# eladhoffer/convNet.pytorch

Hardware: AMD Instinct MI355X
Metric: images/sec ResNet-50 bf16 3x224x224 b=256/GPU training (fwd+bwd+SGD) (higher is better)
Workload: dtype bf16; 1 GPU; ResNet-50 (depth:50) synthetic 3x224x224 b=256/GPU bf16, SGD+momentum, 1 MI355X; global_batch=256, parallelism=dp1

## Files before the change

### convnet.pytorch_amd/csrc/junction.hip

```cpp
#include "cn_common.h"
#include "cn_api_internal.h"
#include <type_traits>

struct JdParams {
  const char* dy;
  const char* w;
  const char* addend;
  const char* bn_y;
  const unsigned char* bn_mask;
  const float* bn_coef;
  char* g;
  float* partial;
  int M, m_per_split, nsplit;
  int co_total;
  int addend_sub, H, W, add_H, add_W;
  FastDiv div_hw, div_w;
  unsigned int dy_bytes, out_bytes, add_bytes, mask_bytes;
};

template <typename T, int KD, int CO>
__global__ __launch_bounds__(512) void jdgrad_kernel(JdParams p) {
  static_assert(sizeof(T) == 2, "16-bit storage");
  constexpr int NCW = CO / 64;
  static_assert(NCW == 4 || NCW == 8, "256 or 512 output channels");
// ... 123 lines not shown
      if (m < m_end) {
        float fv[8], fa[8], yv[8];
        Chunk<T>::unpack(v0, fv);
        Chunk<T>::unpack(ep.a[k], fa);
        Chunk<T>::unpack(ep.y[k], yv);
#pragma unroll
        for (int e = 0; e < 8; ++e) fv[e] += fa[e];
        const unsigned int bits = ep.bits[k];
#pragma unroll
        for (int e = 0; e < 8; ++e) fv[e] = ((bits >> e) & 1u) ? fv[e] : 0.f;
        const u32x4 v = Chunk<T>::pack(fv);
        Chunk<T>::unpack(v, fv);
#pragma unroll
        for (int e = 0; e < 8; ++e) {
          bs1[e] += fv[e];
          bs2[e] = fmaf(fv[e], yv[e], bs2[e]);
        }
        cn_st16(p.g + ((size_t)m * COT + (size_t)cb) * 2, v);
      }
    }
    cn_wave_sync();
  };

  if (m_begin < m_end) {
    Epi cur, nxt;
    load_dy(m_begin);
    load_epi(m_begin, cur);
    int buf = 0;
    for (int mb = m_begin; mb < m_end; mb += BM) {
      store_dy(buf);
      __syncthreads();
      const bool more = mb + BM < m_end;
      if (more) { load_dy(mb + BM); load_epi(mb + BM, nxt); }
      compute(mb, buf, cur);
      if (more) cur = nxt;
      buf ^= 1;
    }
  }
  float r1[8], r2[8];
#pragma unroll
  for (int e = 0; e < 8; ++e) {
    const float mu = p.bn_coef[cb + e], is = p.bn_coef[COT + cb + e];
    r1[e] = bs1[e];
    r2[e] = is * (bs2[e] - mu * bs1[e]);
  }
#pragma unroll
  for (int e = 0; e < 8; ++e)
#pragma unroll
    for (int msk = 8; msk <= 32; msk <<= 1) {
      r1[e] += cn_shfl_xor(r1[e], msk);
      r2[e] += cn_shfl_xor(r2[e], msk);
    }
  __syncthreads();
  float* red = (float*)lds;
  if (lane < 8) {
#pragma unroll
    for (int e = 0; e < 8; ++e) {
      red[(wave * 64 + lane * 8 + e) * 2] = r1[e];
      red[(wave * 64 + lane * 8 + e) * 2 + 1] = r2[e];
    }
  }
  __syncthreads();
  if (tid < CO) {
    const int c = tid, wcol = c / 64, cc = c % 64;
    float a1 = 0.f, a2 = 0.f;
#pragma unroll
// ... 176 lines not shown
    for (int e = 0; e < 8; ++e) {
      dst[cb + e] = r1[e];
      dst[COT + cb + e] = r2[e];
    }
  }
}

static int jd_splits(long long M, int BM) {
  int ns = cn_get_option("jdgrad_splits", 256);
  if (ns < 1) ns = 1;
  const long long stages = (M + BM - 1) / BM;
  if (ns > stages) ns = (int)stages;
  return ns;
}
static int jd_bm(int C) { return C == 256 ? 64 : 32; }
static int jd_plan(long long M, int BM, long long* mps_out, int slices = 1) {
  int ns0 = jd_splits(M, BM);
  if (slices > 1) { ns0 = (ns0 + slices - 1) / slices; if (ns0 < 1) ns0 = 1; }
  long long mps = (M + ns0 - 1) / ns0;
  mps = (mps + BM - 1) / BM * BM;
  if (mps_out != nullptr) *mps_out = mps;
  return (int)((M + mps - 1) / mps);
}

extern "C" int cn_conv2d_dgrad_junction_ok(int C, int K, int dtype) {
  if (dtype != CN_BF16 && dtype != CN_F16) return 0;
  if ((C == 512 || C == 1024) && K == 256) return 1;
  return ((C == 256 && (K == 64 || K == 128)) || (C == 512 && K == 128)) ? 1 : 0;
}
extern "C" int cn_conv2d_dgrad_junction_rows_k(int N, int H, int W, int C, int K) {
  return jd_plan((long long)N * H * W, jd_bm(C), nullptr, K >= 256 ? C / 256 : 1);
}

extern "C" cn_status cn_conv2d_dgrad_junction(const void* dy, const void* w_crsk, void* g, const void* addend, int addend_sub,
                                              int N, int H, int W, int C, int K, int dtype, const void* bn_y,
                                              const unsigned char* bn_mask, const float* bn_coef, float* partial,
                                              int partial_rows, void* stream) {
  if (!cn_conv2d_dgrad_junction_ok(C, K, dtype)) { cn_set_error("conv2d_dgrad_junction: K=%d -> C=%d dtype %d is not an instantiated shape", K, C, dtype); return CN_ESHAPE; }
  if (dy == nullptr || w_crsk == nullptr || g == nullptr || addend == nullptr || bn_y == nullptr || bn_mask == nullptr ||
      bn_coef == nullptr || partial == nullptr) { cn_set_error("conv2d_dgrad_junction: null operand"); return CN_EINVAL; }
  if (addend_sub != 1 && addend_sub != 2) { cn_set_error("conv2d_dgrad_junction: addend subsampling %d (1 or 2)", addend_sub); return CN_EINVAL; }
  const long long M = (long long)N * H * W;
  if (M <= 0) { cn_set_error("conv2d_dgrad_junction: empty"); return CN_ESHAPE; }
  const long long ob = M * C * 2, db = M * K * 2;
  const int aH = (H + 1) / 2, aW = (W + 1) / 2;
  const long long ab = addend_sub == 2 ? (long long)N * aH * aW * C * 2 : ob;
  if (ob >= (1ll << 31) || db >= (1ll << 31)) { cn_set_error("conv2d_dgrad_junction: operand exceeds the 2 GiB buffer-descriptor window"); return CN_ESHAPE; }
  const int BM = jd_bm(C);
  const bool w32 = K >= 256;
  long long mps = 0;
  const int nsplit = jd_plan(M, BM, &mps, w32 ? C / 256 : 1);
  if (partial_rows < nsplit) { cn_set_error("conv2d_dgrad_junction: partial buffer of %d rows < %d", partial_rows, nsplit); return CN_EWORKSPACE; }
  JdParams p;
  memset(&p, 0, sizeof(p));
  p.dy = (const char*)dy; p.w = (const char*)w_crsk; p.addend = (const char*)addend; p.bn_y = (const char*)bn_y;
  p.bn_mask = bn_mask; p.bn_coef = bn_coef; p.g = (char*)g; p.partial = partial;
  p.M = (int)M; p.m_per_split = (int)mps; p.nsplit = nsplit;
  p.co_total = C;
  p.addend_sub = addend_sub; p.H = H; p.W = W; p.add_H = aH; p.add_W = aW;
  p.div_hw = cn_make_fastdiv((unsigned)(H * W)); p.div_w = cn_make_fastdiv((unsigned)W);
  p.dy_bytes = (unsigned int)db; p.out_bytes = (unsigned int)ob; p.add_bytes = (unsigned int)ab;
  hipStream_t st = (hipStream_t)stream;
  const char* tn = dtype == CN_F16 ? "f16_t" : "bf16_t";
  if (w32) {
    cn_set_last_kernel("jdgrad_w32_kernel<%s, %d> [%d channels]", tn, K, C);
    dim3 g32((unsigned)nsplit, (unsigned)(C / 256));
    if (dtype == CN_F16) CN_LAUNCH((jdgrad_w32_kernel<f16_t, 256>), g32, dim3(512), st, p);
    else CN_LAUNCH((jdgrad_w32_kernel<bf16_t, 256>), g32, dim3(512), st, p);
    return cn_check_launch("jdgrad_w32");
  }
  cn_set_last_kernel("jdgrad_kernel<%s, %d, %d>", tn, K, C);
  dim3 grid((unsigned)nsplit, (unsigned)(C > 512 ? C / 512 : 1));
#define JD_GO(KD, CO)                                                                           \
  do {                                                                                          \
    if (dtype == CN_F16) CN_LAUNCH((jdgrad_kernel<f16_t, KD, CO>), grid, dim3(512), st, p);      \
    else CN_LAUNCH((jdgrad_kernel<bf16_t, KD, CO>), grid, dim3(512), st, p);                     \
  } while (0)
  if (C == 256 && K == 64) JD_GO(64, 256);
  else if (C == 256 && K == 128) JD_GO(128, 256);
  else JD_GO(128, 512);
#undef JD_GO
  return cn_check_launch("jdgrad");
}

struct JfParams {
  const char* x;
  const char* w;
  char* y;
  float* partial;
  int M, m_per_split, nsplit;
  int co_total;
  unsigned int x_bytes;
  const float* xf;
  char* a_out;
  int relu;
};

template <typename T, int KD, int CO, bool XF = false>
__global__ __launch_bounds__(512) void jfwd_kernel(JfParams p) {
  static_assert(sizeof(T) == 2, "16-bit storage");
  constexpr int NCW = CO / 64;
  static_assert(NCW == 4 || NCW == 8, "256 or 512 output channels");
  constexpr int PH = 8 / NCW;
  constexpr int BM = 32 * PH;
  constexpr int NKK = KD / 16;
  constexpr int NCD = KD / 8;
  constexpr int DYB = BM * KD * 2;
  constexpr int ND = BM * NCD / 512;
  static_assert(ND >= 1 && BM * NCD % 512 == 0, "x tile staging");
  constexpr int PP = 144;
  constexpr int PRIV = 32 * PP;
  __shared__ __attribute__((aligned(16))) char lds[2 * DYB + 8 * PRIV];
  const int tid = threadIdx.x;
  const int lane = tid & 63;
  const int wave = cn_uniform(tid >> 6);
// ... 352 lines not shown
```

### convnet.pytorch_amd/flags.py

```python
import os

INFINITY_CACHE_BYTES = 256 * 2 ** 20
LAZY_MIN_BYTES = 0.6 * INFINITY_CACHE_BYTES

_DEFAULTS = {
    'fuse_bn_stats': 1,
    'fuse_bn_bwd': 1,
    'fuse_stem_pool': 1,
    'stem_xmax': 1,
    'subsampled_shortcut_grad': 1,
    'dual_bn': 1,
    'lazy_dy': 1,
    'lazy_min_mb': LAZY_MIN_BYTES / 2 ** 20,
    'lazy_z': 1,
    'lazy_a': '1',
    'jpair': 1,
    'jpair_recompute': 1,
    'jdgrad': 1,
    'centered_stats': '1',
    'stem_pairs': 1, 'stem_halo': 1, 'conv3x3_halo': 1, 'conv1x1_stream': 1,
    'dwconv': 1,
    'wgrad_stream': 1,
    'side_hold': 1,
    'dgrad_first': 1,
    'marks': 1,
    'main_stream_prio': '-1',
    'graph': 'auto',
    'graph_dp': 0,
    'plan': 1,
    'quant_int8': 0,
    'quant_fuse': 1,
    'quant_qp_from_producer': 1,
    'quant_store8': 1,
    'quant_wgrad_side': 1,
    'quant_junction_add': 1,
}

_ENV = 'CONVNET_AMD_FLAGS'


def _parse():
    vals = dict(_DEFAULTS)
    for item in os.environ.get(_ENV, '').split(','):
        item = item.strip()
        if not item:
            continue
        name, _, v = item.partition('=')
        if name not in vals:
            raise ValueError('%s: unknown flag %r (known: %s)' % (_ENV, name, ', '.join(sorted(vals))))
        vals[name] = v
    return vals
# ... 28 lines not shown
```

### convnet.pytorch_amd/ops.py

```python
import collections
import contextlib
import os
import typing
import weakref

import torch
import torch.distributed as dist
from torch.autograd import Function

from . import _lib, flags
from ._lib import dtype_code, ptr, stream_of

_WS = {}


def workspace(nbytes, device, tag='main'):
    dev = torch.device(device)
    sid = torch.cuda.current_stream(dev).cuda_stream if dev.type == 'cuda' else 0
    key = (str(dev), tag, sid)
    buf = _WS.get(key)
    if buf is None or buf.numel() * 4 < nbytes:
        n = max(int(nbytes + 3) // 4, 1024)
        old = buf
        buf = torch.empty(n, dtype=torch.float32, device=dev)
# ... 180 lines not shown
def conv_out_hw(H, W, R, S, stride, pad):
    return (H + 2 * pad[0] - R) // stride[0] + 1, (W + 2 * pad[1] - S) // stride[1] + 1



FUSE_BN_STATS = flags.on('fuse_bn_stats')
STEM_PAIRS = flags.on('stem_pairs')
STEM_HALO = flags.on('stem_halo')
CONV3X3_HALO = flags.on('conv3x3_halo')
CONV1X1_STREAM = flags.on('conv1x1_stream')
FUSE_STEM_POOL = flags.on('fuse_stem_pool')
FUSE_BN_BWD = flags.on('fuse_bn_bwd')
LAZY_DY = flags.on('lazy_dy')
LAZY_DY_MIN_MB = float(flags.get('lazy_min_mb'))
DUAL_BN = flags.on('dual_bn')
LAZY_Z = flags.on('lazy_z')
LAZY_Z_MIN_MB = float(flags.get('lazy_min_mb'))
LAZY_Z_SCOPE = [0]
JPAIR = flags.on('jpair')
JPAIR_RECOMPUTE = flags.on('jpair_recompute')
_BN_Y_PRODUCER = [None]


@contextlib.contextmanager
def bn_y_is_output_of(w_krsc):
    prev, _BN_Y_PRODUCER[0] = _BN_Y_PRODUCER[0], w_krsc
    try:
        yield
    finally:
        _BN_Y_PRODUCER[0] = prev


JDGRAD = flags.on('jdgrad')
DGRAD_FIRST = flags.on('dgrad_first')


COUNTERS = {'bn_fwd_fused': 0, 'bn_fwd_plain': 0, 'bn_bwd_fused': 0, 'bn_bwd_plain': 0, 'bn_bwd_lazy': 0}


class _PendingStats(object):
    __slots__ = ('partial', 'rows', 'pivot')


def _stats_partial(want, K, device, rows_fn, *dims):
    if not want:
        return None, 0
    rows = rows_fn(*dims)
    return torch.empty((rows, 2 * K), dtype=torch.float32, device=device), rows


def _park_stats(y, partial, rows, pivot=None):
    if partial is None:
        return
    ps = _PendingStats()
    ps.partial, ps.rows = partial, rows
    ps.pivot = pivot.data_ptr() if pivot is not None else None
    y._cn_stats = ps


def take_pending_stats(y):
    ps = getattr(y, '_cn_stats', None)
    if ps is not None:
        del y._cn_stats
    return ps


# ... 180 lines not shown
            and conv.out_channels <= 128 and conv.in_channels <= 512 and conv.training
            and not getattr(conv, 'out_f32', False))


def conv2d_dgrad(dy, w_crsk, x_shape, K, R, S, stride, pad, addend=None, bn=None, addend_sub=1):
    N, H, W, C = x_shape
    dx = torch.empty((N, H, W, C), dtype=dy.dtype, device=dy.device)
    name = _last_kernel()
    detail = _conv_detail('dgrad', C, H, K, R, stride)
    flops = 2.0 * dy.numel() * C * R * S
    nbytes = dy.numel() * _esize(dy) + dx.numel() * _esize(dx) + K * R * S * C * _esize(dy) \
        + (addend.numel() * _esize(addend) if addend is not None else 0)
    if addend is not None and addend_sub == 2:
        assert tuple(addend.shape) == (N, (H + 1) // 2, (W + 1) // 2, C), 'subsampled addend shape'
    if bn is None and addend is None and _halo3x3_ok(dy, K, C, R, S, stride, pad) and tuple(dy.shape[1:3]) == (H, W):
        PROFILER.run(name, 1, flops, nbytes,
                     lambda: _L().cn_conv3x3_c64(ptr(dy), ptr(w_crsk), ptr(dx), N, H, W, dtype_code(dy.dtype), 1, None,
                                                 0, stream_of(dy)),
                     dy.device, detail=detail)
        return dx
    if bn is None:
        PROFILER.run(name, stride[0] * stride[1], flops, nbytes,
                     lambda: _L().cn_conv2d_dgrad_sa(ptr(dy), ptr(w_crsk), ptr(dx), ptr(addend), int(addend_sub), N, H,
                                                     W, C, K, R, S, stride[0], stride[1], pad[0], pad[1],
                                                     dtype_code(dy.dtype), 0, stream_of(dy)),
                     dy.device, detail=detail)
        return dx
    bn_y, bn_mask, bn_stats, bn_relu = BnBwdOperands(*bn)
    L = _L()
    if JDGRAD and (R, S) == (1, 1) and tuple(stride) == (1, 1) and tuple(pad) == (0, 0) and bn_mask is not None \
            and addend is not None and L.cn_conv2d_dgrad_junction_ok(C, K, dtype_code(dy.dtype)):
        rows = L.cn_conv2d_dgrad_junction_rows_k(N, H, W, C, K)
        partial = torch.empty((rows, 2 * C), dtype=torch.float32, device=dy.device)
        PROFILER.run(_last_kernel(), 1, flops, nbytes + dx.numel() * _esize(dx) + partial.numel() * 4,
                     lambda: L.cn_conv2d_dgrad_junction(ptr(dy), ptr(w_crsk), ptr(dx), ptr(addend), int(addend_sub), N,
                                                        H, W, C, K, dtype_code(dy.dtype), ptr(bn_y), ptr(bn_mask),
                                                        ptr(bn_stats), ptr(partial), rows, stream_of(dy)),
                     dy.device, detail=detail)
        COUNTERS['jdgrad'] = COUNTERS.get('jdgrad', 0) + 1
        return dx, partial, rows
    rows = L.cn_conv2d_dgrad_bnbwd_rows(N, H, W, C, stride[0], stride[1])
    partial = torch.empty((rows, 2 * C), dtype=torch.float32, device=dy.device)
    PROFILER.run(name, stride[0] * stride[1], flops, nbytes + dx.numel() * _esize(dx) + partial.numel() * 4,
                 lambda: L.cn_conv2d_dgrad_bnbwd_sa(ptr(dy), ptr(w_crsk), ptr(dx), ptr(addend), int(addend_sub), N, H,
                                                    W, C, K, R, S, stride[0], stride[1], pad[0], pad[1],
                                                    dtype_code(dy.dtype), ptr(bn_y), ptr(bn_mask), ptr(bn_stats),
                                                    int(bn_relu), ptr(partial), rows, stream_of(dy)),
                 dy.device, detail=detail)
    return dx, partial, rows


def _wgrad_two_phase(call, device, flops, bytes_partial, bytes_reduce, detail, suffix=''):
    if not (PROFILER.enabled and device.type == 'cuda'):
        return call()
    L = _L()
    L.cn_set_option(b'wgrad_phase', 1)
    try:
        PROFILER.run(_last_kernel(suffix), 1, flops, bytes_partial, call, device, detail=detail)
        L.cn_set_option(b'wgrad_phase', 2)
        PROFILER.run('wgrad_reduce_kernel', 1, 0.0, bytes_reduce, call, device, detail=detail + ' [reduce]')
    finally:
        L.cn_set_option(b'wgrad_phase', 0)


def conv2d_wgrad(x, dy, dw_krsc, c_real, K, R, S, stride, pad, beta=1.0, scale=1.0, tag='main'):
    N, H, W, C = x.shape
    code = dtype_code(x.dtype)
    L = _L()
    need = L.cn_conv2d_wgrad_workspace(N, H, W, C, K, R, S, stride[0], stride[1], pad[0], pad[1], code)
    ws = workspace(need, x.device, tag)

# ... 325 lines not shown
    _L().cn_cast_from_f32(ptr(x), ptr(y), x.numel(), dtype_code(dtype), stream_of(x))
    return y


def fill_f32_(x, v=0.0):
    _L().cn_fill_f32(ptr(x), x.numel(), float(v), stream_of(x))
    return x



def _input_bn_state(conv_mod, x):
    bn_mod = getattr(conv_mod, 'input_bn', None)
    if bn_mod is None:
        return None
    ref = getattr(bn_mod, '_fwd_ctx', None)
    bctx = ref() if ref is not None else None
    if bctx is None or getattr(bctx, 'out_ptr', None) != x.data_ptr():
        return None
    try:
        saved = bctx.saved_tensors
    except RuntimeError:
        return None
    y, stats = saved[0], saved[1]
    mask = saved[2] if len(saved) > 2 else None
    if tuple(y.shape) != tuple(x.shape) or y.dtype != x.dtype:
        return None
    if bctx.has_res and bctx.relu and mask is None:
        return None
    if y.shape[-1] % _lib.chunk_elems(y.dtype) != 0:
        return None
    return bn_mod, BnBwdOperands(y, mask, stats, bctx.relu)


_ZEROS = {}


def _zero_like_placeholder(x):
    key = (x.device, x.dtype)
    z = _ZEROS.get(key)
    if z is None:
        z = _ZEROS[key] = torch.zeros(1, dtype=x.dtype, device=x.device)
    return z.expand(x.shape)


def _is_zero_placeholder(t):
    z = _ZEROS.get((t.device, t.dtype))
    return z is not None and t.data_ptr() == z.data_ptr() and t.dim() > 0 and all(st == 0 for st in t.stride())


def _submit_wgrad(mod, run, held, dy):
    x = held[0]
    if SIDE.active(x):
        SIDE.submit(x.device, lambda: held + (run('side') or ()), mod._notify_grad_ready, dy)
    else:
        run('main')
        mod._notify_grad_ready()


class Conv2dFunction(Function):
    @staticmethod
    def forward(ctx, x, weight, bias, mod):
        mod.ensure_prepared()
        lz, la = _take(mod, '_lazy_z', x), _take(mod, '_lazy_a', x)
        if bias is not None and (lz is not None or la is not None):
            raise _lib.ConvNetHipError(_MISMATCH['_lazy_z' if lz is not None else '_lazy_a'])
        if lz is not None:
            y = conv2d_fwd_lazyz(lz, mod.w_krsc, mod.out_channels, bn_stats=_wants_stats(mod), pivot=stats_pivot(mod))
            COUNTERS['lazy_z'] = COUNTERS.get('lazy_z', 0) + 1
        elif la is not None:
            y = conv2d_fwd_lazya(la, mod.w_krsc, mod.out_channels, bn_stats=_wants_stats(mod), kernel=mod.kernel_size)
            COUNTERS['lazy_a'] = COUNTERS.get('lazy_a', 0) + 1
        else:
            y = conv2d_fwd(x, mod.w_krsc, bias, mod.out_channels, mod.kernel_size[0], mod.kernel_size[1],
                           mod.stride, mod.padding, out_f32=mod.out_f32, bn_stats=_wants_stats(mod),
                           pivot=stats_pivot(mod))
        ctx.mod = mod
        ctx.has_bias = bias is not None
        ctx.save_for_backward(x)
        ctx.out_key = _owner_key(y)
        _take(mod, '_lazy_dy')
        return y

    @staticmethod
    def backward(ctx, dy):
        (x,) = ctx.saved_tensors
        mod = ctx.mod
        lazy = _take(mod, '_lazy_dy', ctx.out_key)
        holder = getattr(mod, '_res_holder', None)
        R, S = mod.kernel_size
        if lazy is None and _is_zero_placeholder(dy):
            raise _lib.ConvNetHipError('lazy dy: the gradient placeholder reached a convolution with an empty mailbox '
                                       '(the BatchNorm that parked the gradient is not this convolution\'s consumer)')
        if lazy is not None:
            g, bn_y, coef = lazy
            if tuple(g.shape) != tuple(dy.shape):
                raise _lib.ConvNetHipError(_MISMATCH['_lazy_dy'])
            if JPAIR and (R, S) == (1, 1) and mod.stride == (1, 1) and mod.padding == (0, 0) and ctx.needs_input_grad[0] \
                    and mod.in_channels == x.shape[-1] \
                    and _L().cn_conv2d_bwd1x1_lazy_ok(x.shape[-1], mod.out_channels, dtype_code(x.dtype)):
                if holder is not None and holder.dres is not None:
                    raise _lib.ConvNetHipError('lazy dy met a fused-addend dgrad: the junction layout changed')
                own = JPAIR_RECOMPUTE and not ctx.has_bias and _owner_key(bn_y) == ctx.out_key
                with bn_y_is_output_of(mod.w_krsc if own else None):
                    dx = conv2d_bwd1x1_lazy(x, g, bn_y, coef, mod.w_crsk, mod.grad_view('weight'), mod.out_channels)
                mod._notify_grad_ready()
                COUNTERS['jpair'] = COUNTERS.get('jpair', 0) + 1
                if holder is not None:
                    holder.park(dx)
                return dx, None, None, None
            _submit_wgrad(mod, lambda tag: conv2d_wgrad_lazy(x, g, bn_y, coef, mod.grad_view('weight'), mod.in_channels,
                                                             mod.out_channels, R, S, mod.stride, mod.padding, tag=tag),
                          (x, g, bn_y, coef), coef)
            if not ctx.needs_input_grad[0]:
# ... 12 lines not shown
                holder.park(dx)
            return dx, None, None, None
        dy = dy.contiguous()
        if dy.dtype != x.dtype:
            dy = cast_from_f32(dy, x.dtype)
        if ctx.has_bias:
            colsum(dy.view(-1, mod.out_channels), mod.grad_view('bias'))

        def submit_wgrad():
            _submit_wgrad(mod, lambda tag: conv2d_wgrad(x, dy, mod.grad_view('weight'), mod.in_channels, mod.out_channels,
                                                        R, S, mod.stride, mod.padding, tag=tag), (x, dy), dy)

        def dgrad_part():
            dx = None
            if ctx.needs_input_grad[0]:
                addend, addend_sub = None, 1
                if holder is not None and holder.dres is not None and holder.dres.dtype == dy.dtype \
                        and (holder.dres.shape == x.shape if holder.sub == 1 else
                             tuple(holder.dres.shape) == (x.shape[0], (x.shape[1] + 1) // 2, (x.shape[2] + 1) // 2, x.shape[3])):
                    addend, addend_sub = holder.claim()
                elif holder is not None and holder.dres is None and SUBSAMPLED_SHORTCUT_GRAD \
                        and (R, S) == (1, 1) and mod.stride == (2, 2) and mod.padding == (0, 0):
                    N_, H_, W_, C_ = x.shape
                    compact = conv2d_dgrad(dy, mod.w_crsk, (N_, (H_ + 1) // 2, (W_ + 1) // 2, C_), mod.out_channels, 1, 1,
                                           (1, 1), (0, 0))
                    holder.park(compact, 2)
                    return _zero_like_placeholder(x), None, None, None
                final = holder is None or addend is not None
                bn_args = _input_bn_state(mod, x) if (final and FUSE_BN_BWD) else None
                if bn_args is not None and holder is None:
                    bn_args = None
                if bn_args is not None:
                    bn_mod, bn = bn_args
                    dx, partial, rows = conv2d_dgrad(dy, mod.w_crsk, x.shape, mod.out_channels, R, S, mod.stride,
                                                     mod.padding, addend=addend, bn=bn, addend_sub=addend_sub)
                    _park(bn_mod, '_bwd_partials', dx, BwdPartials(partial, rows))
                else:
                    dx = conv2d_dgrad(dy, mod.w_crsk, x.shape, mod.out_channels, R, S, mod.stride, mod.padding,
                                      addend=addend, addend_sub=addend_sub)
                if holder is not None and addend is None:
                    holder.park(dx)
            return dx, None, None, None

        if not DGRAD_FIRST:
            submit_wgrad()
        out = dgrad_part()
        if DGRAD_FIRST:
            submit_wgrad()
        return out


class GroupedConv2dFunction(Function):
    @staticmethod
    def forward(ctx, x, weight, mod):
        mod.ensure_prepared()
        _refuse_parked(mod, 'grouped convolution')
        y = gconv2d_fwd(x, mod.w_krsc, mod.out_channels, mod.groups, mod.stride[0])
        ctx.mod = mod
        ctx.save_for_backward(x)
        COUNTERS['gconv'] = COUNTERS.get('gconv', 0) + 1
        return y

    @staticmethod
    def backward(ctx, dy):
        (x,) = ctx.saved_tensors
        mod = ctx.mod
        _refuse_parked(mod, 'grouped convolution')
        if _is_zero_placeholder(dy):
# ... 845 lines not shown
```

### include/convnet_hip.h

```cpp
#ifndef CONVNET_HIP_H
#define CONVNET_HIP_H
#include <stddef.h>
#ifdef __cplusplus
extern "C" {
#endif

#define CN_OK 0
#define CN_EINVAL (-1)
#define CN_ESHAPE (-2)
#define CN_EHIP (-3)
#define CN_EWORKSPACE (-4)
#define CN_ERCCL (-5)
#define CN_F32 0
#define CN_BF16 1
#define CN_F16 2
typedef int cn_status;

const char* cn_last_error(void);
const char* cn_build_info(void);
const char* cn_last_kernel_name(void);
const char* cn_kernel_log(int clear);
int cn_is_emulator(void);
int cn_set_option(const char* name, int value);
cn_status cn_stream_fork(void* from_stream, void* to_stream);
// ... 31 lines not shown
cn_status cn_conv3x3_c64_lazya(const void* bn_y, const float* stats, int relu, void* a_out, const void* w, void* y, int N, int H,
                               int W, int dtype, float* partial, int partial_rows, void* stream);
int cn_stem_fwd_ok(int K, int R, int S2, int Jp, int dtype);
int cn_stem_fwd_rows(int N, int P);
cn_status cn_stem_fwd(const void* xp, const void* wp, void* y, int N, int Hp, int Jp, int dtype, float* partial,
                      int partial_rows, void* stream);
int cn_stem_wgrad_ok(int K, int R, int S2, int Jp, int dtype);
size_t cn_stem_wgrad_workspace(int N, int Hp);
cn_status cn_stem_wgrad(const void* xp, const void* dy, float* dwp, int N, int Hp, int Jp, int dtype, float beta, float scale,
                        void* workspace, size_t ws_bytes, void* stream);
cn_status cn_conv2d_fwd_lazyz(const void* bn_y, const void* res, const float* stats, const float* res_stats, int relu, void* z,
                              unsigned char* z_mask, const void* w_krsc, void* y, int N, int H, int W, int C, int K, int dtype,
                              float* partial, int partial_rows, const float* pivot, void* stream);
int cn_conv2d_dgrad_bnbwd_rows(int N, int H, int W, int C, int stride_h, int stride_w);
cn_status cn_conv2d_dgrad_sa(const void* dy, const void* w_crsk, void* dx, const void* addend, int addend_sub, int N, int H,
                             int W, int C, int K, int R, int S, int stride_h, int stride_w, int pad_h, int pad_w, int dtype,
                             int out_f32, void* stream);
cn_status cn_conv2d_dgrad_bnbwd_sa(const void* dy, const void* w_crsk, void* g, const void* addend, int addend_sub, int N,
                                   int H, int W, int C, int K, int R, int S, int stride_h, int stride_w, int pad_h, int pad_w,
                                   int dtype, const void* bn_y, const unsigned char* bn_mask, const float* bn_coef,
                                   int bn_relu, float* partial, int partial_rows, void* stream);
int cn_conv1x1_stream_fwd_ok(int C, int K, int dtype);
int cn_conv1x1_stream_fwd_rows(int N, int H, int W, int K);
cn_status cn_conv1x1_stream_fwd(const void* x, const void* w_krsc, void* y, int N, int H, int W, int C, int K, int dtype,
                                float* partial, int partial_rows, void* stream);
cn_status cn_conv1x1_stream_fwd_lazya(const void* bn_y, const float* stats, int relu, void* a_out, const void* w_krsc, void* y,
                                      int N, int H, int W, int C, int K, int dtype, float* partial, int partial_rows,
                                      void* stream);
int cn_conv2d_dgrad_junction_ok(int C, int K, int dtype);
int cn_conv2d_dgrad_junction_rows_k(int N, int H, int W, int C, int K);
cn_status cn_conv2d_dgrad_junction(const void* dy, const void* w_crsk, void* g, const void* addend, int addend_sub, int N, int H,
                                   int W, int C, int K, int dtype, const void* bn_y, const unsigned char* bn_mask,
                                   const float* bn_coef, float* partial, int partial_rows, void* stream);
int cn_gconv2d_ok(int C, int K, int groups, int R, int S, int stride_h, int stride_w, int pad_h, int pad_w, int dtype);
cn_status cn_gconv2d_fwd(const void* x, const void* w, void* y, int N, int H, int W, int C, int K, int groups, int stride,
                         int dtype, void* stream);
cn_status cn_gconv2d_dgrad(const void* dy, const void* w, void* dx, int N, int H, int W, int C, int K, int groups, int stride,
                           int dtype, void* stream);
size_t cn_gconv2d_wgrad_workspace(int N, int H, int W, int C, int K, int groups, int stride, int dtype);
cn_status cn_gconv2d_wgrad(const void* x, const void* dy, float* dw, int N, int H, int W, int C, int K, int groups, int stride,
                           int dtype, float beta, float scale, void* workspace, size_t ws_bytes, void* stream);
int cn_dwconv3x3_ok(int C, int R, int S, int stride_h, int stride_w, int pad_h, int pad_w, int dtype);
cn_status cn_dwconv3x3_fwd(const void* x, const void* w_rsc, const float* bias, void* y, int N, int H, int W, int C, int stride,
                           int dtype, void* stream);
cn_status cn_dwconv3x3_dgrad(const void* dy, const void* w_rsc, void* dx, int N, int H, int W, int C, int stride, int dtype,
                             void* stream);
size_t cn_dwconv3x3_wgrad_workspace(int N, int H, int W, int C, int stride, int dtype);
cn_status cn_dwconv3x3_wgrad(const void* x, const void* dy, float* dw, float* dbias, int N, int H, int W, int C, int stride,
                             int dtype, float beta, float scale, void* workspace, size_t ws_bytes, void* stream);
size_t cn_conv2d_wgrad_workspace(int N, int H, int W, int C, int K, int R, int S, int stride_h, int stride_w,
                                 int pad_h, int pad_w, int dtype);
cn_status cn_conv2d_wgrad(const void* x, const void* dy, float* dw_krsc, int C_real, int N, int H, int W, int C,
                          int K, int R, int S, int stride_h, int stride_w, int pad_h, int pad_w, int dtype,
                          float beta, float scale, void* workspace, size_t ws_bytes, void* stream);
cn_status cn_conv2d_dgrad_lazy(const void* g, const void* bn_y, const float* coef, const void* w_crsk, void* dx, int N, int H,
                               int W, int C, int K, int R, int S, int stride_h, int stride_w, int pad_h, int pad_w, int dtype,
                               void* stream);
cn_status cn_conv2d_wgrad_lazy(const void* x, const void* g, const void* bn_y, const float* coef, float* dw_krsc, int C_real,
                               int N, int H, int W, int C, int K, int R, int S, int stride_h, int stride_w, int pad_h,
                               int pad_w, int dtype, float beta, float scale, void* workspace, size_t ws_bytes, void* stream);
int cn_conv2d_dgrad_lazy_stream_ok(int C, int K, int dtype);
cn_status cn_conv2d_dgrad_lazy_stream(const void* g, const void* bn_y, const float* coef, const void* w_crsk, void* dx, int N,
                                      int H, int W, int C, int K, int dtype, void* stream);
int cn_conv2d_bwd1x1_lazy_ok(int C, int K, int dtype);
size_t cn_conv2d_bwd1x1_lazy_workspace(int N, int H, int W, int C, int K);
cn_status cn_conv2d_bwd1x1_lazy(const void* x, const void* g, const void* bn_y, const float* coef, const void* w_crsk, void* dx,
// ... 244 lines not shown
```

Baseline: 15080 images/sec.

## Recompute BN input from 1x1 producer conv inside junction dgrad kernel

Adds a jdgrad_kernel_ry variant that recomputes the BatchNorm input y on the fly as a 1x1 convolution of the saved 64-channel producer input, instead of reading the stored 256-channel bn_y tensor. The Python side detects when the BN's producer is a bias-free 1x1 conv with 64 input channels and routes through the new path by default. This trades extra MFMA work and LDS staging of the producer weights for reading a narrower tensor from HBM. It also lets bn_y avoid being materialized or read in the backward pass for those layers.

```diff
diff --git a/convnet.pytorch_amd/csrc/junction.hip b/convnet.pytorch_amd/csrc/junction.hip
--- a/convnet.pytorch_amd/csrc/junction.hip
+++ b/convnet.pytorch_amd/csrc/junction.hip
@@ -179,6 +179,287 @@
       __syncthreads();
       const bool more = mb + BM < m_end;
       if (more) { load_dy(mb + BM); load_epi(mb + BM, nxt); }
+      compute(mb, buf, cur);
+      if (more) cur = nxt;
+      buf ^= 1;
+    }
+  }
+  float r1[8], r2[8];
+#pragma unroll
+  for (int e = 0; e < 8; ++e) {
+    const float mu = p.bn_coef[cb + e], is = p.bn_coef[COT + cb + e];
+    r1[e] = bs1[e];
+    r2[e] = is * (bs2[e] - mu * bs1[e]);
+  }
+#pragma unroll
+  for (int e = 0; e < 8; ++e)
+#pragma unroll
+    for (int msk = 8; msk <= 32; msk <<= 1) {
+      r1[e] += cn_shfl_xor(r1[e], msk);
+      r2[e] += cn_shfl_xor(r2[e], msk);
+    }
+  __syncthreads();
+  float* red = (float*)lds;
+  if (lane < 8) {
+#pragma unroll
+    for (int e = 0; e < 8; ++e) {
+      red[(wave * 64 + lane * 8 + e) * 2] = r1[e];
+      red[(wave * 64 + lane * 8 + e) * 2 + 1] = r2[e];
+    }
+  }
+  __syncthreads();
+  if (tid < CO) {
+    const int c = tid, wcol = c / 64, cc = c % 64;
+    float a1 = 0.f, a2 = 0.f;
+#pragma unroll
+    for (int g2 = 0; g2 < PH; ++g2) {
+      a1 += red[((g2 * NCW + wcol) * 64 + cc) * 2];
+      a2 += red[((g2 * NCW + wcol) * 64 + cc) * 2 + 1];
+    }
+    float* dst = p.partial + (size_t)split * 2 * COT;
+    dst[co0 + c] = a1;
+    dst[COT + co0 + c] = a2;
+  }
+}
+
+struct JdRyParams {
+  JdParams j;
+  const char* px;
+  const char* pw;
+  unsigned int px_bytes;
+};
+
+template <typename T, int KD, int CO, int KX>
+__global__ __launch_bounds__(512) void jdgrad_kernel_ry(JdRyParams q) {
+  static_assert(sizeof(T) == 2, "16-bit storage");
+  const JdParams& p = q.j;
+  constexpr int NCW = CO / 64;
+  static_assert(NCW == 4 || NCW == 8, "256 or 512 output channels");
+  constexpr int PH = 8 / NCW;
+  constexpr int BM = 32 * PH;
+  constexpr int NKK = KD / 16;
+  constexpr int NCD = KD / 8;
+  constexpr int DYB = BM * KD * 2;
+  constexpr int ND = BM * NCD / 512;
+  static_assert(ND >= 1 && BM * NCD % 512 == 0, "dy tile staging");
+  constexpr int NKX = KX / 16;
+  constexpr int NCX = KX / 8;
+  constexpr int XB = BM * KX * 2;
+  constexpr int NX = BM * NCX / 512;
+  static_assert(NX >= 1 && BM * NCX % 512 == 0 && NCX >= 8, "px tile staging");
+  constexpr int PP = 144;
+  constexpr int PRIV = 32 * PP;
+  constexpr bool WL = KD > 64;
+  constexpr int WLB = WL ? CO * KX * 2 : 0;
+  __shared__ __attribute__((aligned(16))) char lds[2 * DYB + 2 * XB + 8 * PRIV + WLB];
+  const int tid = threadIdx.x;
+  const int lane = tid & 63;
+  const int wave = cn_uniform(tid >> 6);
+  const int cw = wave % NCW, ph = wave / NCW;
+  const int h = lane >> 5;
+  char* xt = lds + 2 * DYB;
+  char* priv = lds + 2 * DYB + 2 * XB + wave * PRIV;
+  char* wl = lds + 2 * DYB + 2 * XB + 8 * PRIV;
+
+  const int split = blockIdx.x;
+  const int co0 = blockIdx.y * CO, COT = p.co_total;
+  const int m_begin = split * p.m_per_split;
+  int m_end = m_begin + p.m_per_split;
+  if (m_end > p.M) m_end = p.M;
+
+  s16x8 wf[2][NKK], wy[2][WL ? 1 : NKX];
+#pragma unroll
+  for (int t = 0; t < 2; ++t) {
+    const int c = co0 + cw * 64 + t * 32 + (lane & 31);
+#pragma unroll
+    for (int kk = 0; kk < NKK; ++kk)
+      wf[t][kk] = __builtin_bit_cast(s16x8, cn_ld16(p.w + ((size_t)c * KD + 16 * kk + 8 * h) * 2));
+    if constexpr (!WL) {
+#pragma unroll
+      for (int kk = 0; kk < NKX; ++kk)
+        wy[t][kk] = __builtin_bit_cast(s16x8, cn_ld16(q.pw + ((size_t)c * KX + 16 * kk + 8 * h) * 2));
+    }
+  }
+  if constexpr (WL) {
+    for (int id = tid; id < CO * NCX; id += 512) {
+      const int row = id / NCX, c = id - row * NCX;
+      const int cs = NCX == 8 ? (c ^ ((row >> 1) & 7)) : (c ^ (row & (NCX - 1)));
+      cn_st16(wl + row * (KX * 2) + (cs << 4), cn_ld16(q.pw + ((size_t)(co0 + row) * KX + (size_t)c * 8) * 2));
+    }
+  }
+
+  const cn_buf_t dybuf = cn_make_buf(p.dy, p.dy_bytes);
+  const cn_buf_t abuf = cn_make_buf(p.addend, p.add_bytes);
+  const cn_buf_t xbuf = cn_make_buf(q.px, q.px_bytes);
+  const int ech = lane & 7, erow = lane >> 3;
+  const int cb = co0 + cw * 64 + ech * 8;
+  const int HW = p.H * p.W;
+
+  struct Epi {
+    u32x4 a[4];
+    unsigned int bits[4];
+  };
+  u32x4 dreg[ND], xreg[NX];
+  auto load_tiles = [&](int mb) {
+#pragma unroll
+    for (int i = 0; i < ND; ++i) {
+      const int id = tid + 512 * i;
+      const int row = id / NCD, c = id - row * NCD;
+      const int m = mb + row;
+      dreg[i] = cn_buf_ld16(dybuf, m < m_end ? ((unsigned int)m * (unsigned int)KD + (unsigned int)c * 8u) * 2u : CN_OOB);
+    }
+#pragma unroll
+    for (int i = 0; i < NX; ++i) {
+      const int id = tid + 512 * i;
+      const int row = id / NCX, c = id - row * NCX;
+      const int m = mb + row;
+      xreg[i] = cn_buf_ld16(xbuf, m < m_end ? ((unsigned int)m * (unsigned int)KX + (unsigned int)c * 8u) * 2u : CN_OOB);
+    }
+  };
+  auto load_epi = [&](int mb, Epi& e) {
+#pragma unroll
+    for (int k = 0; k < 4; ++k) {
+      const int m = mb + ph * 32 + k * 8 + erow;
+      const bool ok = m < m_end;
+      unsigned int oa = ok ? ((unsigned int)m * (unsigned int)COT + (unsigned int)cb) * 2u : CN_OOB;
+      if (p.addend_sub == 2) {
+        const int mm = ok ? m : 0;
+        const int n = (int)cn_fastdiv((unsigned)mm, p.div_hw);
+        const int rem = mm - n * HW;
+        const int ho = (int)cn_fastdiv((unsigned)rem, p.div_w);
+        const int wo = rem - ho * p.W;
+        const bool even = ((ho | wo) & 1) == 0;
+        const int apx = (n * p.add_H + (ho >> 1)) * p.add_W + (wo >> 1);
+        oa = (ok && even) ? ((unsigned int)apx * (unsigned int)COT + (unsigned int)cb) * 2u : CN_OOB;
+      }
+      e.a[k] = cn_buf_ld16(abuf, oa);
+      e.bits[k] = ok ? (unsigned int)p.bn_mask[(size_t)m * (COT / 8) + (cb >> 3)] : 0u;
+    }
+  };
+  auto store_tiles = [&](int buf) {
+    char* t = lds + buf * DYB;
+#pragma unroll
+    for (int i = 0; i < ND; ++i) {
+      const int id = tid + 512 * i;
+      const int row = id / NCD, c = id - row * NCD;
+      const int cs = NCD == 8 ? (c ^ ((row >> 1) & 7)) : (c ^ (row & (NCD - 1)));
+      cn_st16(t + row * (KD * 2) + (cs << 4), dreg[i]);
+    }
+    char* u = xt + buf * XB;
+#pragma unroll
+    for (int i = 0; i < NX; ++i) {
+      const int id = tid + 512 * i;
+      const int row = id / NCX, c = id - row * NCX;
+      const int cs = NCX == 8 ? (c ^ ((row >> 1) & 7)) : (c ^ (row & (NCX - 1)));
+      cn_st16(u + row * (KX * 2) + (cs << 4), xreg[i]);
+    }
+  };
+
+  float bs1[8], bs2[8];
+#pragma unroll
+  for (int e = 0; e < 8; ++e) { bs1[e] = 0.f; bs2[e] = 0.f; }
+
+  auto compute = [&](int mb, int buf, const Epi& ep) {
+    const int prow = ph * 32 + (lane & 31);
+    f32x16 acc[2];
+#pragma unroll
+    for (int x = 0; x < 2; ++x)
+#pragma unroll
+      for (int r = 0; r < 16; ++r) acc[x][r] = 0.f;
+    {
+      const char* rowp = lds + buf * DYB + prow * (KD * 2);
+      const int sw = NCD == 8 ? ((prow >> 1) & 7) : (prow & (NCD - 1));
+#pragma unroll
+      for (int kk = 0; kk < NKK; ++kk) {
+        const s16x8 b = __builtin_bit_cast(s16x8, cn_ld16(rowp + (((2 * kk + h) ^ sw) << 4)));
+#pragma unroll
+        for (int x = 0; x < 2; ++x) {
+          if constexpr (std::is_same<T, f16_t>::value) acc[x] = cn_mfma_32x32x16_f16(wf[x][kk], b, acc[x]);
+          else acc[x] = cn_mfma_32x32x16_bf16(wf[x][kk], b, acc[x]);
+        }
+      }
+    }
+    auto to_patch = [&]() {
+#pragma unroll
+      for (int x = 0; x < 2; ++x)
+#pragma unroll
+        for (int q4 = 0; q4 < 4; ++q4) {
+          u32x2 pk;
+          pk[0] = cn_pack2<T>(acc[x][q4 * 4], acc[x][q4 * 4 + 1]);
+          pk[1] = cn_pack2<T>(acc[x][q4 * 4 + 2], acc[x][q4 * 4 + 3]);
+          *(u32x2*)(priv + (lane & 31) * PP + (x * 32 + 8 * q4 + 4 * h) * 2) = pk;
+        }
+    };
+    to_patch();
+    cn_wave_sync();
+    u32x4 v0[4];
+#pragma unroll
+    for (int k = 0; k < 4; ++k) v0[k] = cn_ld16(priv + (k * 8 + erow) * PP + ech * 16);
+    cn_wave_sync();
+#pragma unroll
+    for (int x = 0; x < 2; ++x)
+#pragma unroll
+      for (int r = 0; r < 16; ++r) acc[x][r] = 0.f;
+    {
+      const char* rowp = xt + buf * XB + prow * (KX * 2);
+      const int sw = NCX == 8 ? ((prow >> 1) & 7) : (prow & (NCX - 1));
+#pragma unroll
+      for (int kk = 0; kk < NKX; ++kk) {
+        const s16x8 b = __builtin_bit_cast(s16x8, cn_ld16(rowp + (((2 * kk + h) ^ sw) << 4)));
+#pragma unroll
+        for (int x = 0; x < 2; ++x) {
+          s16x8 a;
+          if constexpr (WL) {
+            const int wrow = cw * 64 + x * 32 + (lane & 31);
+            const int ws = NCX == 8 ? ((wrow >> 1) & 7) : (wrow & (NCX - 1));
+            a = __builtin_bit_cast(s16x8, cn_ld16(wl + wrow * (KX * 2) + (((2 * kk + h) ^ ws) << 4)));
+          } else {
+            a = wy[x][kk];
+          }
+          if constexpr (std::is_same<T, f16_t>::value) acc[x] = cn_mfma_32x32x16_f16(a, b, acc[x]);
+          else acc[x] = cn_mfma_32x32x16_bf16(a, b, acc[x]);
+        }
+      }
+    }
+    to_patch();
+    cn_wave_sync();
+#pragma unroll
+    for (int k = 0; k < 4; ++k) {
+      const int m = mb + ph * 32 + k * 8 + erow;
+      const u32x4 y0 = cn_ld16(priv + (k * 8 + erow) * PP + ech * 16);
+      if (m < m_end) {
+        float fv[8], fa[8], yv[8];
+        Chunk<T>::unpack(v0[k], fv);
+        Chunk<T>::unpack(ep.a[k], fa);
+        Chunk<T>::unpack(y0, yv);
+#pragma unroll
+        for (int e = 0; e < 8; ++e) fv[e] += fa[e];
+        const unsigned int bits = ep.bits[k];
+#pragma unroll
+        for (int e = 0; e < 8; ++e) fv[e] = ((bits >> e) & 1u) ? fv[e] : 0.f;
+        const u32x4 v = Chunk<T>::pack(fv);
+        Chunk<T>::unpack(v, fv);
+#pragma unroll
+        for (int e = 0; e < 8; ++e) {
+          bs1[e] += fv[e];
+          bs2[e] = fmaf(fv[e], yv[e], bs2[e]);
+        }
+        cn_st16(p.g + ((size_t)m * COT + (size_t)cb) * 2, v);
+      }
+    }
+    cn_wave_sync();
+  };
+
+  if (m_begin < m_end) {
+    Epi cur, nxt;
+    load_tiles(m_begin);
+    load_epi(m_begin, cur);
+    int buf = 0;
+    for (int mb = m_begin; mb < m_end; mb += BM) {
+      store_tiles(buf);
+      __syncthreads();
+      const bool more = mb + BM < m_end;
+      if (more) { load_tiles(mb + BM); load_epi(mb + BM, nxt); }
       compute(mb, buf, cur);
       if (more) cur = nxt;
       buf ^= 1;
@@ -421,12 +702,12 @@
   return jd_plan((long long)N * H * W, jd_bm(C), nullptr, K >= 256 ? C / 256 : 1);
 }
 
-extern "C" cn_status cn_conv2d_dgrad_junction(const void* dy, const void* w_crsk, void* g, const void* addend, int addend_sub,
-                                              int N, int H, int W, int C, int K, int dtype, const void* bn_y,
-                                              const unsigned char* bn_mask, const float* bn_coef, float* partial,
-                                              int partial_rows, void* stream) {
+static cn_status jd_run(const void* dy, const void* w_crsk, void* g, const void* addend, int addend_sub, int N, int H, int W,
+                        int C, int K, int dtype, const void* bn_y, const void* prod_x, const void* prod_w_krsc, int KX,
+                        const unsigned char* bn_mask, const float* bn_coef, float* partial, int partial_rows, void* stream) {
+  const bool ry = bn_y == nullptr;
   if (!cn_conv2d_dgrad_junction_ok(C, K, dtype)) { cn_set_error("conv2d_dgrad_junction: K=%d -> C=%d dtype %d is not an instantiated shape", K, C, dtype); return CN_ESHAPE; }
-  if (dy == nullptr || w_crsk == nullptr || g == nullptr || addend == nullptr || bn_y == nullptr || bn_mask == nullptr ||
+  if (dy == nullptr || w_crsk == nullptr || g == nullptr || addend == nullptr || (ry && (prod_x == nullptr || prod_w_krsc == nullptr)) || bn_mask == nullptr ||
       bn_coef == nullptr || partial == nullptr) { cn_set_error("conv2d_dgrad_junction: null operand"); return CN_EINVAL; }
   if (addend_sub != 1 && addend_sub != 2) { cn_set_error("conv2d_dgrad_junction: addend subsampling %d (1 or 2)", addend_sub); return CN_EINVAL; }
   const long long M = (long long)N * H * W;
@@ -434,7 +715,7 @@
   const long long ob = M * C * 2, db = M * K * 2;
   const int aH = (H + 1) / 2, aW = (W + 1) / 2;
   const long long ab = addend_sub == 2 ? (long long)N * aH * aW * C * 2 : ob;
-  if (ob >= (1ll << 31) || db >= (1ll << 31)) { cn_set_error("conv2d_dgrad_junction: operand exceeds the 2 GiB buffer-descriptor window"); return CN_ESHAPE; }
+  if (ob >= (1ll << 31) || db >= (1ll << 31) || (ry && M * KX * 2 >= (1ll << 31))) { cn_set_error("conv2d_dgrad_junction: operand exceeds the 2 GiB buffer-descriptor window"); return CN_ESHAPE; }
   const int BM = jd_bm(C);
   const bool w32 = K >= 256;
   long long mps = 0;
@@ -451,6 +732,22 @@
   p.dy_bytes = (unsigned int)db; p.out_bytes = (unsigned int)ob; p.add_bytes = (unsigned int)ab;
   hipStream_t st = (hipStream_t)stream;
   const char* tn = dtype == CN_F16 ? "f16_t" : "bf16_t";
+  if (ry) {
+    JdRyParams q;
+    memset(&q, 0, sizeof(q));
+    q.j = p; q.px = (const char*)prod_x; q.pw = (const char*)prod_w_krsc; q.px_bytes = (unsigned int)(M * KX * 2);
+    cn_set_last_kernel("jdgrad_kernel_ry<%s, %d, %d, %d>", tn, K, C, KX);
+    dim3 grid((unsigned)nsplit);
+#define JD_GO(KD, CO, KXX)                                                                         \
+  do {                                                                                             \
+    if (dtype == CN_F16) CN_LAUNCH((jdgrad_kernel_ry<f16_t, KD, CO, KXX>), grid, dim3(512), st, q); \
+    else CN_LAUNCH((jdgrad_kernel_ry<bf16_t, KD, CO, KXX>), grid, dim3(512), st, q);                \
+  } while (0)
+    if (K == 64) JD_GO(64, 256, 64);
+    else JD_GO(128, 256, 64);
+#undef JD_GO
+    return cn_check_launch("jdgrad_ry");
+  }
   if (w32) {
     cn_set_last_kernel("jdgrad_w32_kernel<%s, %d> [%d channels]", tn, K, C);
     dim3 g32((unsigned)nsplit, (unsigned)(C / 256));
@@ -470,6 +767,27 @@
   else JD_GO(128, 512);
 #undef JD_GO
   return cn_check_launch("jdgrad");
+}
+extern "C" cn_status cn_conv2d_dgrad_junction(const void* dy, const void* w_crsk, void* g, const void* addend, int addend_sub,
+                                              int N, int H, int W, int C, int K, int dtype, const void* bn_y,
+                                              const unsigned char* bn_mask, const float* bn_coef, float* partial,
+                                              int partial_rows, void* stream) {
+  if (bn_y == nullptr) { cn_set_error("conv2d_dgrad_junction: null operand"); return CN_EINVAL; }
+  return jd_run(dy, w_crsk, g, addend, addend_sub, N, H, W, C, K, dtype, bn_y, nullptr, nullptr, 0, bn_mask, bn_coef, partial,
+                partial_rows, stream);
+}
+extern "C" int cn_conv2d_dgrad_junction_ry_ok(int C, int K, int KX, int dtype) {
+  if (dtype != CN_BF16 && dtype != CN_F16) return 0;
+  return (C == 256 && (K == 64 || K == 128) && KX == 64) ? 1 : 0;
+}
+extern "C" cn_status cn_conv2d_dgrad_junction_ry(const void* dy, const void* w_crsk, void* g, const void* addend, int addend_sub,
+                                                 int N, int H, int W, int C, int K, int KX, int dtype, const void* prod_x,
+                                                 const void* prod_w_krsc, const unsigned char* bn_mask, const float* bn_coef,
+                                                 float* partial, int partial_rows, void* stream) {
+  if (!cn_conv2d_dgrad_junction_ry_ok(C, K, KX, dtype)) { cn_set_error("conv2d_dgrad_junction_ry: K=%d -> C=%d from KX=%d dtype %d is not an instantiated shape", K, C, KX, dtype); return CN_ESHAPE; }
+  if (prod_x == nullptr || prod_w_krsc == nullptr) { cn_set_error("conv2d_dgrad_junction_ry: null operand"); return CN_EINVAL; }
+  return jd_run(dy, w_crsk, g, addend, addend_sub, N, H, W, C, K, dtype, nullptr, prod_x, prod_w_krsc, KX, bn_mask, bn_coef,
+                partial, partial_rows, stream);
 }
 
 struct JfParams {
diff --git a/convnet.pytorch_amd/flags.py b/convnet.pytorch_amd/flags.py
--- a/convnet.pytorch_amd/flags.py
+++ b/convnet.pytorch_amd/flags.py
@@ -17,6 +17,7 @@
     'jpair': 1,
     'jpair_recompute': 1,
     'jdgrad': 1,
+    'jdgrad_recompute': 1,
     'centered_stats': '1',
     'stem_pairs': 1, 'stem_halo': 1, 'conv3x3_halo': 1, 'conv1x1_stream': 1,
     'dwconv': 1,
diff --git a/convnet.pytorch_amd/ops.py b/convnet.pytorch_amd/ops.py
--- a/convnet.pytorch_amd/ops.py
+++ b/convnet.pytorch_amd/ops.py
@@ -236,6 +236,19 @@
 
 
 JDGRAD = flags.on('jdgrad')
+JDGRAD_RECOMPUTE = flags.on('jdgrad_recompute')
+_BN_Y_CONV1X1 = [None]
+
+
+@contextlib.contextmanager
+def bn_y_is_conv1x1_of(prod_x, prod_w_krsc):
+    prev, _BN_Y_CONV1X1[0] = _BN_Y_CONV1X1[0], (prod_x, prod_w_krsc) if prod_x is not None else None
+    try:
+        yield
+    finally:
+        _BN_Y_CONV1X1[0] = prev
+
+
 DGRAD_FIRST = flags.on('dgrad_first')
 
 
@@ -482,11 +495,28 @@
             and addend is not None and L.cn_conv2d_dgrad_junction_ok(C, K, dtype_code(dy.dtype)):
         rows = L.cn_conv2d_dgrad_junction_rows_k(N, H, W, C, K)
         partial = torch.empty((rows, 2 * C), dtype=torch.float32, device=dy.device)
-        PROFILER.run(_last_kernel(), 1, flops, nbytes + dx.numel() * _esize(dx) + partial.numel() * 4,
-                     lambda: L.cn_conv2d_dgrad_junction(ptr(dy), ptr(w_crsk), ptr(dx), ptr(addend), int(addend_sub), N,
-                                                        H, W, C, K, dtype_code(dy.dtype), ptr(bn_y), ptr(bn_mask),
-                                                        ptr(bn_stats), ptr(partial), rows, stream_of(dy)),
-                     dy.device, detail=detail)
+        prod = _BN_Y_CONV1X1[0]
+        if prod is not None and L.cn_conv2d_dgrad_junction_ry_ok(C, K, prod[0].shape[-1], dtype_code(dy.dtype)):
+            px, pw = prod
+            KX = px.shape[-1]
+            if px.numel() != N * H * W * KX or pw.numel() != C * KX or px.dtype != dy.dtype or pw.dtype != dy.dtype \
+                    or not px.is_contiguous() or not pw.is_contiguous():
+                raise _lib.ConvNetHipError('conv2d_dgrad: bn_y_is_conv1x1_of operands do not describe a %d -> %d channel '
+                                           '1x1 convolution over this input' % (KX, C))
+            PROFILER.run(_last_kernel(), 1, flops + 2.0 * px.numel() * C,
+                         nbytes + (px.numel() + pw.numel()) * _esize(px) + partial.numel() * 4,
+                         lambda: L.cn_conv2d_dgrad_junction_ry(ptr(dy), ptr(w_crsk), ptr(dx), ptr(addend), int(addend_sub),
+                                                               N, H, W, C, K, KX, dtype_code(dy.dtype), ptr(px), ptr(pw),
+                                                               ptr(bn_mask), ptr(bn_stats), ptr(partial), rows,
+                                                               stream_of(dy)),
+                         dy.device, detail=detail)
+            COUNTERS['jdgrad_ry'] = COUNTERS.get('jdgrad_ry', 0) + 1
+        else:
+            PROFILER.run(_last_kernel(), 1, flops, nbytes + dx.numel() * _esize(dx) + partial.numel() * 4,
+                         lambda: L.cn_conv2d_dgrad_junction(ptr(dy), ptr(w_crsk), ptr(dx), ptr(addend), int(addend_sub), N,
+                                                            H, W, C, K, dtype_code(dy.dtype), ptr(bn_y), ptr(bn_mask),
+                                                            ptr(bn_stats), ptr(partial), rows, stream_of(dy)),
+                         dy.device, detail=detail)
         COUNTERS['jdgrad'] = COUNTERS.get('jdgrad', 0) + 1
         return dx, partial, rows
     rows = L.cn_conv2d_dgrad_bnbwd_rows(N, H, W, C, stride[0], stride[1])
@@ -878,6 +908,31 @@
     return bn_mod, BnBwdOperands(y, mask, stats, bctx.relu)
 
 
+def _bn_y_producer(bn_mod, bn_y):
+    conv = getattr(bn_mod, 'producer_conv', None)
+    if not JDGRAD_RECOMPUTE or conv is None:
+        return None, None
+    ref = conv.__dict__.get('_fwd_ctx')
+    pctx = ref() if ref is not None else None
+    if pctx is None or getattr(pctx, 'mod', None) is not conv or getattr(pctx, 'has_bias', True) \
+            or getattr(pctx, 'out_key', None) != _owner_key(bn_y):
+        return None, None
+    if getattr(conv, 'kernel_size', None) != (1, 1) or getattr(conv, 'stride', None) != (1, 1) \
+            or getattr(conv, 'padding', None) != (0, 0) or getattr(conv, 'groups', 1) != 1 \
+            or getattr(conv, 'bias', None) is not None:
+        return None, None
+    if conv.in_channels != 64 or conv.out_channels != bn_y.shape[-1] or bn_y.dtype not in (torch.bfloat16, torch.float16):
+        return None, None
+    try:
+        (px,) = pctx.saved_tensors
+    except RuntimeError:
+        return None, None
+    if px.dtype != bn_y.dtype or not px.is_contiguous() or tuple(px.shape[:-1]) != tuple(bn_y.shape[:-1]) \
+            or px.shape[-1] != conv.in_channels:
+        return None, None
+    return px, conv.w_krsc
+
+
 _ZEROS = {}
 
 
@@ -925,6 +980,7 @@
         ctx.save_for_backward(x)
         ctx.out_key = _owner_key(y)
         _take(mod, '_lazy_dy')
+        mod._fwd_ctx = weakref.ref(ctx)
         return y
 
     @staticmethod
@@ -1003,8 +1059,9 @@
                     bn_args = None
                 if bn_args is not None:
                     bn_mod, bn = bn_args
-                    dx, partial, rows = conv2d_dgrad(dy, mod.w_crsk, x.shape, mod.out_channels, R, S, mod.stride,
-                                                     mod.padding, addend=addend, bn=bn, addend_sub=addend_sub)
+                    with bn_y_is_conv1x1_of(*_bn_y_producer(bn_mod, bn.y)):
+                        dx, partial, rows = conv2d_dgrad(dy, mod.w_crsk, x.shape, mod.out_channels, R, S, mod.stride,
+                                                         mod.padding, addend=addend, bn=bn, addend_sub=addend_sub)
                     _park(bn_mod, '_bwd_partials', dx, BwdPartials(partial, rows))
                 else:
                     dx = conv2d_dgrad(dy, mod.w_crsk, x.shape, mod.out_channels, R, S, mod.stride, mod.padding,
diff --git a/include/convnet_hip.h b/include/convnet_hip.h
--- a/include/convnet_hip.h
+++ b/include/convnet_hip.h
@@ -87,6 +87,11 @@
 cn_status cn_conv2d_dgrad_junction(const void* dy, const void* w_crsk, void* g, const void* addend, int addend_sub, int N, int H,
                                    int W, int C, int K, int dtype, const void* bn_y, const unsigned char* bn_mask,
                                    const float* bn_coef, float* partial, int partial_rows, void* stream);
+int cn_conv2d_dgrad_junction_ry_ok(int C, int K, int KX, int dtype);
+cn_status cn_conv2d_dgrad_junction_ry(const void* dy, const void* w_crsk, void* g, const void* addend, int addend_sub, int N,
+                                      int H, int W, int C, int K, int KX, int dtype, const void* prod_x,
+                                      const void* prod_w_krsc, const unsigned char* bn_mask, const float* bn_coef,
+                                      float* partial, int partial_rows, void* stream);
 int cn_gconv2d_ok(int C, int K, int groups, int R, int S, int stride_h, int stride_w, int pad_h, int pad_w, int dtype);
 cn_status cn_gconv2d_fwd(const void* x, const void* w, void* y, int N, int H, int W, int C, int K, int groups, int stride,
                          int dtype, void* stream);
```

Result: no change. 15100 images/sec, median of 5 (+0.1%).
